# chorowski-lab/pytorch-asr

Hardware: AMD Instinct MI355X
Metric: CTC train-step frames/sec (higher is better)
Workload: dtype bf16; 1 GPU; WSJ mono-char CTC (egs/wsj/yamls/ctc.yaml shapes), DeepSpeech2 conv+4xBiLSTM-320 encoder + FSTDecoder, fwd+bwd+GradientClipping(clip 480000, skip 4.8e+06 = recipe x global_batch/16)+PolyakDecay+Adam, synthetic 40-dim x 1-channel x 1000-frame fbank; batch_per_gpu=768, global_batch=768, frames=1000, classes=49, parallelism=dp1, batch_norm=per-replica statistics, optimizer_steps=139, step_boundary=device: att_speech.fused_step (clip / skip decision + Adam, no read-back)

## Files before the change

pytorch-asr_amd/csrc/conv.hip:

```cpp
#include <type_traits>
#include "common.h"
#include "../../include/asr_amd.h"

namespace {

typedef __attribute__((ext_vector_type(8))) __bf16 bf16x8;
typedef __attribute__((ext_vector_type(16))) float f32x16;
typedef __attribute__((ext_vector_type(4))) unsigned int u32x4;
typedef __attribute__((ext_vector_type(4))) float f32x4;
typedef __attribute__((ext_vector_type(4))) __bf16 bf16x4;

constexpr int CH = 32;
constexpr int KS = 7;
constexpr int PIX = 80;
constexpr int KSTEPS = KS * KS * CH / 16;

typedef __attribute__((ext_vector_type(4))) int rsrc_words;
__device__ __forceinline__ rsrc_words conv_raw_rsrc(const void *base, unsigned bytes) {
    const unsigned long long a = (unsigned long long)base;
    rsrc_words r;
    r.x = __builtin_amdgcn_readfirstlane((int)(unsigned)a);
    r.y = __builtin_amdgcn_readfirstlane((int)((unsigned)(a >> 32) & 0xffffu));
    r.z = __builtin_amdgcn_readfirstlane((int)bytes);
    r.w = 0x00020000;
    return r;
}
__device__ __forceinline__ void conv_dma16(rsrc_words r, unsigned lds_byte, unsigned voff, unsigned soff) {
    unsigned keep;
    asm volatile("s_mov_b32 %0, m0\n\ts_mov_b32 m0, %1\n\ts_nop 0\n\t"
                 "buffer_load_dwordx4 %2, %3, %4 offen lds\n\ts_mov_b32 m0, %0"
                 : "=&s"(keep)
                 : "s"(lds_byte), "v"(voff), "s"(r), "s"(soff)
                 : "memory");
}
__device__ __forceinline__ unsigned conv_lds_addr(const void *ptr) {
    return (unsigned)(size_t)((__attribute__((address_space(3))) const void *)ptr);
}

inline int pick_row_pitch(int min_pitch, int per_row, int step, int npix, int ntiles) {
    static const int grp[2][16] = {{0, 1, 2, 3, 12, 13, 14, 15, 20, 21, 22, 23, 24, 25, 26, 27},
                                   {4, 5, 6, 7, 8, 9, 10, 11, 16, 17, 18, 19, 28, 29, 30, 31}};
    int best = min_pitch, best_cost = 1 << 30;
    for (int P = min_pitch; P <= min_pitch + 256; P += 16) {
        int cost = 0;
        for (int tile = 0; tile < ntiles; ++tile)
            for (int g = 0; g < 2; ++g) {
                int addr_of_bank[64], worst = 1, cnt[64];
                for (int b = 0; b < 64; ++b) { addr_of_bank[b] = -1; cnt[b] = 0; }
                for (int i = 0; i < 16; ++i) {
                    int m = 32 * tile + grp[g][i];
                    if (m >= npix) m = npix - 1;
                    const int r = m / per_row, w = m - r * per_row;
                    const int a = r * step * P + w * PIX;
                    for (int k = 0; k < 4; ++k) {
                        const int b = (a / 4 + k) & 63;
                        if (addr_of_bank[b] != a + 4 * k) {
                            addr_of_bank[b] = a + 4 * k;
                            if (++cnt[b] > worst) worst = cnt[b];
                        }
                    }
                }
                cost += worst;
            }
        if (cost < best_cost) { best_cost = cost; best = P; }
    }
    return best;
}

inline int conv_cu_count() {
    int dev = 0, cus = 0;
    if (hipGetDevice(&dev) != hipSuccess) return 0;
    if (hipDeviceGetAttribute(&cus, hipDeviceAttributeMultiprocessorCount, dev) != hipSuccess) return 0;
    return cus;
}

__device__ __forceinline__ void chan_partial_sums(const __bf16 *oimg, int npix, float *red, float *partial) {
    const int tid = threadIdx.x, ch = tid & 31, grp = tid >> 5;
    float s = 0.f, q = 0.f;
    int m = grp;
    for (; m + 56 < npix; m += 64) {
        float v[8];
#pragma unroll
        for (int u = 0; u < 8; ++u) v[u] = (float)oimg[(m + 8 * u) * CH + ch];
#pragma unroll
        for (int u = 0; u < 8; ++u) {
            s += v[u];
            q += v[u] * v[u];
        }
    }
    for (; m < npix; m += 8) {
        const float v = (float)oimg[m * CH + ch];
        s += v;
        q += v * v;
    }
    red[grp * 64 + ch] = s;
    red[grp * 64 + 32 + ch] = q;
    __syncthreads();
    if (tid < 64) {
        float t = 0.f;
#pragma unroll
        for (int g = 0; g < 8; ++g) t += red[g * 64 + tid];
        partial[tid] = t;
    }
}

__global__ __launch_bounds__(1024) void chan_sums_reduce_kernel(const float *partial, int nparts, double *out) {
    __shared__ double lds[1024];
    const int el = threadIdx.x & 63, way = threadIdx.x >> 6;
    double s = 0.0;
    for (int g = blockIdx.x * 16 + way; g < nparts; g += gridDim.x * 16) s += (double)partial[(size_t)g * 64 + el];
    lds[way * 64 + el] = s;
    __syncthreads();
    if (way == 0) {
        double t = 0.0;
        for (int w = 0; w < 16; ++w) t += lds[w * 64 + el];
        atomicAdd(out + el, t);
    }
}

__global__ void zero_chan_sums_kernel(double *out) { out[threadIdx.x] = 0.0; }

__global__ void conv_pack_fwd_kernel(const float *w, __bf16 *out) {
    const int i = blockIdx.x * blockDim.x + threadIdx.x;
    if (i >= KSTEPS * 64 * 8) return;
    const int j = i & 7, l = (i >> 3) & 63, s = i >> 9;
    const int k = 16 * s + 8 * (l >> 5) + j, co = l & 31;
    const int tap = k / CH, ci = k % CH, kt = tap / KS, kf = tap % KS;
    out[i] = (__bf16)w[((co * CH + ci) * KS + kt) * KS + kf];
}

#ifdef CONV_STAMPS
#define STAMP(k) do { if (p.stamps && blockIdx.x == 7 && lane == 0 && nst < 64) { p.stamps[(wave * 64 + nst) * 8 + (k)] = (long long)__builtin_amdgcn_s_memtime(); } } while (0)
#else
#define STAMP(k) do { } while (0)
#endif

struct ConvFwdParams {
    long long *stamps;
    const __bf16 *x;
    const __bf16 *wpack;
    __bf16 *y;
    float *stats;
    int B, H, W, Ho, Wo, R;
    int pitch;
};

constexpr int FWD_NT = 2, FWD_PIX = 2 * FWD_NT * 32, FWD_AD = 3;
constexpr int FWD_MAXQ = 15;

// ... 128 lines not shown
                f32x4 v = {c[4 * g], c[4 * g + 1], c[4 * g + 2], c[4 * g + 3]};
                v = KH == 0 ? v + o[g] : o[g] + v;
                bf16x4 o4 = {(__bf16)v[0], (__bf16)v[1], (__bf16)v[2], (__bf16)v[3]};
                *reinterpret_cast<bf16x4 *>(take + wr_off + (((unsigned)g ^ wr_swz) << 4)) = o4;
            }
        }
        asm volatile("" ::: "memory");
        STAMP(6);
        if (item + (int)gridDim.x < nitems) stage(item + gridDim.x, ln);
        const int rows_here = (p.Ho - ho0) < R ? (p.Ho - ho0) : R;
        const int nvalid = rows_here * Wo - 32 * tile;
        if (p.stats) {
            const unsigned ch = (unsigned)ln & 31u;
            const unsigned p0 = (unsigned)(ln >> 5) * 16u;
            float ssum = 0.f, qsum = 0.f;
#pragma unroll
            for (int k = 0; k < 16; ++k) {
                const unsigned pp = p0 + (unsigned)k;
                const unsigned short raw = *reinterpret_cast<const unsigned short *>(
                    take + pp * 64u + ((((ch >> 3) ^ (pp >> 2)) & 3u) << 4) + (ch & 7u) * 2u);
                const float v = (int)pp < nvalid ? __uint_as_float((unsigned)raw << 16) : 0.f;
                ssum += v;
                qsum += v * v;
                if ((k & 3) == 3) asm volatile("" ::: "memory");
            }
            run[ln] += ssum;
            run[64 + ln] += qsum;
        }
        asm volatile("" ::: "memory");
        STAMP(7);
        {
            const char *ybase = reinterpret_cast<const char *>(p.y) + ((size_t)b * p.Ho + ho0) * Wo * 64;
            u32x4 v[2];
#pragma unroll
            for (int it = 0; it < 2; ++it) {
                const unsigned e = (unsigned)(ln + 64 * it);
                v[it] = *reinterpret_cast<const u32x4 *>(take + ((e ^ ((e >> 4) & 3u)) << 4));
            }
#pragma unroll
            for (int it = 0; it < 2; ++it)
                conv_store16(ybase, (unsigned)(rows_here * Wo * 64), v[it], (unsigned)(2048 * tile + 16 * (ln + 64 * it)));
        }
    }
    if (p.stats) {
        const int ln = threadIdx.x & 63;
        const float a0 = run[ln & 31] + run[32 + (ln & 31)], a1 = run[64 + (ln & 31)] + run[96 + (ln & 31)];
        p.stats[((size_t)blockIdx.x * 4 + wave) * 64 + ln] = ln < 32 ? a0 : a1;
    }
}

template <int SH>
__global__ __launch_bounds__(256, 2) void conv7x7c32_fwd_kernel(ConvFwdParams p) {
    extern __shared__ char smem[];
    const int lane = threadIdx.x & 63;
    const int wave = __builtin_amdgcn_readfirstlane(threadIdx.x >> 6);
    if ((wave & 1) == 0) conv_fwd_wave<SH, 0>(p, smem, lane, wave);
    else conv_fwd_wave<SH, 1>(p, smem, lane, wave);
}


__global__ void conv_pack_dgrad_kernel(const float *w, __bf16 *out) {
    const int i = blockIdx.x * blockDim.x + threadIdx.x;
    if (i >= KSTEPS * 64 * 8) return;
    const int jj = i & 7, l = (i >> 3) & 63, s = i >> 9;
    const int r = s < 42 ? 0 : (s < 70 ? 1 : 2);
    const int sl = s - (r == 0 ? 0 : (r == 1 ? 42 : 70));
    const int j = sl / 14, rem = sl % 14, kf = rem >> 1, cp = rem & 1;
    const int co = cp * 16 + 8 * (l >> 5) + jj, ci = l & 31, kt = r + 3 * j;
    out[i] = (__bf16)w[((co * CH + ci) * KS + kt) * KS + kf];
}

struct ConvDgradParams {
    long long *stamps;
    const __bf16 *dy;
    const __bf16 *wpack;
    __bf16 *dx;
    int B, H, W, Ho, Wo, Rq;
    int pitch;
    int flip;
};

constexpr int DG_NT = 6, DG_PIX = DG_NT * 32, DG_AD = 2;

template <int NS, int S0>
__device__ __forceinline__ void conv_dgrad_part(const char *img, const unsigned (&pixbase)[DG_NT], int pitch,
                                                const bf16x8 (&bf)[28], f32x16 (&acc)[DG_NT]) {
    constexpr int N = NS * DG_NT;
    auto frag = [&](int idx) {
        const int s = idx / DG_NT, i = idx % DG_NT;
        const int sl = S0 + s;
        const int j = sl / 14, rem = sl % 14, kf = rem >> 1, cp = rem & 1;
        const unsigned off = (unsigned)((2 - j) * pitch + (6 - kf) * PIX + cp * 32);
        return *reinterpret_cast<const bf16x8 *>(img + pixbase[i] + off);
    };
    bf16x8 a[DG_AD];
#pragma unroll
    for (int d = 0; d < DG_AD; ++d) a[d] = frag(d);
#pragma unroll
    for (int idx = 0; idx < N; ++idx) {
        acc[idx % DG_NT] = __builtin_amdgcn_mfma_f32_32x32x16_bf16(bf[idx / DG_NT], a[idx % DG_AD],
                                                                   idx < DG_NT ? f32x16{} : acc[idx % DG_NT], 0, 0, 0);
        if (idx + DG_AD < N) a[idx % DG_AD] = frag(idx + DG_AD);
    }
#pragma unroll
    for (int d = 0; d < DG_AD; ++d) __builtin_amdgcn_sched_group_barrier(0x100, 1, 0);
#pragma unroll
    for (int idx = 0; idx < N; ++idx) {
        __builtin_amdgcn_sched_group_barrier(0x008, 1, 0);
        if (idx + DG_AD < N) __builtin_amdgcn_sched_group_barrier(0x100, 1, 0);
    }
}

template <int ROLE>
__device__ __forceinline__ void conv_dgrad_wave(const ConvDgradParams &p, char *smem, int lane, int wave) {
    constexpr int NS = ROLE < 2 ? 21 : 28;
    constexpr int FIRST = ROLE == 0 ? 0 : (ROLE == 1 ? 21 : (ROLE == 2 ? 42 : 70));
    constexpr int R = ROLE < 2 ? 0 : ROLE - 1;
    constexpr int HT = DG_NT / 2;
    constexpr int NT = ROLE < 2 ? HT : DG_NT, T0 = ROLE == 1 ? HT : 0;
    constexpr int GIVE0 = ROLE == 0 ? HT : 0;
    constexpr int SLOTS = 14;
    const int W = p.W, Wo = p.Wo, Rq = p.Rq;
    const unsigned img_bytes = (unsigned)(Rq + 2) * (unsigned)p.pitch;
    bf16x8 bf[28];
    {
        const bf16x8 *src = reinterpret_cast<const bf16x8 *>(p.wpack) + (size_t)FIRST * 64 + lane;
#pragma unroll
        for (int s = 0; s < NS; ++s) bf[s] = src[(size_t)s * 64];
    }
    unsigned tab[SLOTS];
    if (ROLE < 2) {
#pragma unroll
        for (int kk = 0; kk < SLOTS; ++kk) {
            const unsigned beta = (unsigned)(SLOTS * ROLE + kk) * 1024u + (unsigned)lane * 16u;
            const unsigned row = beta / (unsigned)p.pitch, rem = beta - row * (unsigned)p.pitch;
            const unsigned col = (rem * 52429u) >> 22, within = rem - col * 80u;
            const int wo = (int)col - 6;
            const bool ok = beta < img_bytes && within < 64u && wo >= 0 && wo < Wo;
            tab[kk] = ok ? (row * (unsigned)Wo + (unsigned)wo) * 64u + within : 0xC0000000u;
        }
    }
    unsigned pixbase[DG_NT];
    const int npix = Rq * W;
#pragma unroll
    for (int i = 0; i < DG_NT; ++i) {
        int m = 32 * i + (lane & 31);
        if (m >= npix) m = npix - 1;
        const int q = m / W, w = m - q * W;
        pixbase[i] = (unsigned)(q * p.pitch + w * PIX + (lane >> 5) * 16);
    }
    const int nq = (p.H + 2) / 3;
    const int tiles = (nq + Rq - 1) / Rq, nitems = tiles * p.B;
    const int nslots = (int)((img_bytes + 1023u) / 1024u);
    constexpr int HALF = HT * 4 * 64 * 16;
    char *epi = smem + nslots * 1024;
    char *part_out = epi + (ROLE == 0 ? 0 : HALF);
    char *part_in = epi + (ROLE == 0 ? HALF : 0);
    char *ocls = ROLE == 0 ? epi + HALF : ROLE == 1 ? epi - T0 * 2048 : epi + 2 * HALF + (R - 1) * DG_PIX * 64;
    const unsigned img_lds = conv_lds_addr(smem);
    const unsigned item_bytes = (unsigned)(p.Ho * Wo * 64);
    auto stage = [&](int it) {
        const int b = it / tiles, q0 = (it - b * tiles) * Rq;
        const rsrc_words yR = conv_raw_rsrc(reinterpret_cast<const char *>(p.dy) + (size_t)b * item_bytes, item_bytes);
        const unsigned base = (unsigned)((q0 - 2) * Wo * 64);
#pragma unroll
        for (int kk = 0; kk < SLOTS; ++kk)
            if (SLOTS * ROLE + kk < nslots)
                conv_dma16(yR, (unsigned)__builtin_amdgcn_readfirstlane((int)(img_lds + (SLOTS * ROLE + kk) * 1024u)),
                           tab[kk] + base, 0u);
    };
    if (ROLE < 2 && (int)blockIdx.x < nitems) stage(blockIdx.x);
    const unsigned wr_base = (unsigned)((lane & 31) * 64 + ((lane >> 5) << 3));
    const unsigned wr_swz = (unsigned)((lane >> 2) & 3);
    const unsigned qmagic = 65536u / (unsigned)W + 1u;
    const int cls_chunks = Rq * W * 4;
    int nst = 0;
    for (int item = blockIdx.x; item < nitems; item += gridDim.x, ++nst) {
        const int b = item / tiles, q0 = (item - b * tiles) * Rq;
        STAMP(0);
        if (ROLE < 2) asm volatile("s_waitcnt vmcnt(0)" ::: "memory");
        __syncthreads();
        f32x16 acc[DG_NT];
        STAMP(1);
        conv_dgrad_part<NS, ROLE == 1 ? 21 : 0>(smem, pixbase, p.pitch, bf, acc);
        STAMP(2);
        if (ROLE < 2) {
#pragma unroll
            for (int i = 0; i < HT; ++i)
#pragma unroll
                for (int g = 0; g < 4; ++g) {
                    const f32x16 &c = acc[GIVE0 + i];
                    *reinterpret_cast<f32x4 *>(part_out + ((i * 4 + g) * 64 + lane) * 16) =
                        f32x4{c[4 * g], c[4 * g + 1], c[4 * g + 2], c[4 * g + 3]};
                }
        }
        STAMP(3);
        __syncthreads();
        STAMP(4);
        if (ROLE < 2 && item + (int)gridDim.x < nitems) stage(item + gridDim.x);
        {
            constexpr int E = NT * 4, RD = ROLE < 2 ? E / 2 : E;
#pragma unroll
            for (int e0 = 0; e0 < E; e0 += RD) {
                f32x4 o[ROLE < 2 ? RD : 1];
                if (ROLE < 2) {
#pragma unroll
                    for (int k = 0; k < RD; ++k)
                        o[k] = *reinterpret_cast<const f32x4 *>(part_in + ((e0 + k) * 64 + lane) * 16);
                    asm volatile("s_waitcnt lgkmcnt(0)" ::: "memory");
                }
#pragma unroll
                for (int k = 0; k < RD; ++k) {
                    const int i = (e0 + k) / 4, g = (e0 + k) % 4;
                    const f32x16 &c = acc[T0 + i];
                    f32x4 v = {c[4 * g], c[4 * g + 1], c[4 * g + 2], c[4 * g + 3]};
                    if (ROLE < 2) v += o[k];
                    bf16x4 o4 = {(__bf16)v[0], (__bf16)v[1], (__bf16)v[2], (__bf16)v[3]};
                    *reinterpret_cast<bf16x4 *>(ocls + (T0 + i) * 2048 + wr_base + (((unsigned)g ^ wr_swz) << 4)) = o4;
                }
            }
        }
        STAMP(5);
        {
            char *xb = reinterpret_cast<char *>(p.dx) + ((size_t)b * p.H + 3 * q0 + R) * W * 64;
            const int qlim = (p.H - R + 2) / 3 - q0;
            int e0 = T0 * 128 + lane;
            asm volatile("" : "+v"(e0));
#pragma unroll
            for (int rd = 0; rd < NT * 2; rd += 6) {
                u32x4 v[6];
#pragma unroll
                for (int it = 0; it < 6; ++it) {
                    const unsigned e = (unsigned)(e0 + 64 * (rd + it)), m = e >> 2;
                    v[it] = *reinterpret_cast<const u32x4 *>(ocls + ((e ^ ((m >> 2) & 3u)) << 4));
                }
#pragma unroll
                for (int it = 0; it < 6; ++it) {
                    const unsigned e = (unsigned)(e0 + 64 * (rd + it)), m = e >> 2, q = (m * qmagic) >> 16;
                    if ((int)e < cls_chunks && (int)q < qlim)
                        *reinterpret_cast<u32x4 *>(xb + (size_t)(e * 16u + q * (unsigned)(2 * W * 64))) = v[it];
                }
            }
        }
        STAMP(6); STAMP(7);
    }
}

__global__ __launch_bounds__(256, 2) void conv7x7c32_dgrad_s3_kernel(ConvDgradParams p) {
    extern __shared__ char smem[];
    const int lane = threadIdx.x & 63;
    const int wave = __builtin_amdgcn_readfirstlane(threadIdx.x >> 6);
    const int role = __builtin_amdgcn_readfirstlane(p.flip && blockIdx.x >= (gridDim.x >> 1) ? 3 - wave : wave);
    if (role == 0) conv_dgrad_wave<0>(p, smem, lane, wave);
    else if (role == 1) conv_dgrad_wave<1>(p, smem, lane, wave);
    else if (role == 2) conv_dgrad_wave<2>(p, smem, lane, wave);
    else conv_dgrad_wave<3>(p, smem, lane, wave);
}


typedef __attribute__((ext_vector_type(4))) short s16x4;
typedef __attribute__((ext_vector_type(8))) short s16x8;
typedef __attribute__((address_space(3))) s16x4 lds_s16x4;

__device__ __forceinline__ bf16x8 tr_frag(const char *addr) {
    const s16x4 lo = __builtin_amdgcn_ds_read_tr16_b64_v4i16((lds_s16x4 *)(addr));
    const s16x4 hi = __builtin_amdgcn_ds_read_tr16_b64_v4i16((lds_s16x4 *)(addr + 4 * PIX));
    s16x8 v;
    v.s0 = lo.x; v.s1 = lo.y; v.s2 = lo.z; v.s3 = lo.w;
    v.s4 = hi.x; v.s5 = hi.y; v.s6 = hi.z; v.s7 = hi.w;
    return __builtin_bit_cast(bf16x8, v);
}

constexpr int WGRAD_WGS = 256;
constexpr int WGRAD_NT = 448;
constexpr int NX_MAX = 8, ND_MAX = 3;

struct ConvWgradParams {
    const __bf16 *x, *dy;
    float *partial;
    int B, H, W, Ho, Wo, KW;
    int rows;
};

__global__ __launch_bounds__(WGRAD_NT) void conv7x7c32_wgrad_s3_kernel(ConvWgradParams p) {
    extern __shared__ char smem[];
    const int tid = threadIdx.x, lane = tid & 63;
    const int wave = __builtin_amdgcn_readfirstlane(tid >> 6);
    const int W = p.W, Wo = p.Wo, KW = p.KW, Wd = 16 * KW, rows = p.rows;
    const int xrows = 3 * (rows - 1) + KS;
    char *ximg = smem;
    char *dimg = smem + (size_t)(xrows * W + 24) * PIX;
    const int kt = wave;
    f32x16 acc[KS];
#pragma unroll
    for (int f = 0; f < KS; ++f)
#pragma unroll
        for (int j = 0; j < 16; ++j) acc[f][j] = 0.f;
    const unsigned lane_off = (unsigned)((8 * (lane >> 5) + ((lane & 15) >> 2)) * PIX +
                                         (16 * ((lane >> 4) & 1) + 4 * (lane & 3)) * 2);
    for (int i = tid; i < 24 * PIX / 4; i += WGRAD_NT)
        reinterpret_cast<unsigned *>(ximg + (size_t)xrows * W * PIX)[i] = 0u;
    const int chunks_per_utt = (p.Ho + rows - 1) / rows;
    const int nchunks = p.B * chunks_per_utt;
    const int nx = xrows * W * 4, nd = rows * Wd * 4;
    u32x4 sx[NX_MAX], sd[ND_MAX];
    const unsigned wmagic = (1u << 20) / (unsigned)W + 1u, dmagic = (1u << 20) / (unsigned)Wd + 1u;
    auto fetch = [&](int c) {
        const int b = c / chunks_per_utt, ho0 = (c - b * chunks_per_utt) * rows;
        const char *xb = reinterpret_cast<const char *>(p.x) + (size_t)b * p.H * W * 64;
        const char *yb = reinterpret_cast<const char *>(p.dy) + (size_t)b * p.Ho * Wo * 64;
#pragma unroll
        for (int k = 0; k < NX_MAX; ++k) {
            const int i = tid + k * WGRAD_NT;
            const int pix = i >> 2, part = i & 3, row = (int)(((unsigned)pix * wmagic) >> 20);
            u32x4 v = {0u, 0u, 0u, 0u};
            if (i < nx && 3 * ho0 + row < p.H)
                v = *reinterpret_cast<const u32x4 *>(xb + ((size_t)(3 * ho0) * W + pix) * 64 + part * 16);
            sx[k] = v;
        }
#pragma unroll
        for (int k = 0; k < ND_MAX; ++k) {
            const int i = tid + k * WGRAD_NT;
            const int pix = i >> 2, part = i & 3, row = (int)(((unsigned)pix * dmagic) >> 20), wo = pix - row * Wd;
            u32x4 v = {0u, 0u, 0u, 0u};
            if (i < nd && ho0 + row < p.Ho && wo < Wo)
                v = *reinterpret_cast<const u32x4 *>(yb + ((size_t)(ho0 + row) * Wo + wo) * 64 + part * 16);
            sd[k] = v;
        }
    };
    auto stage = [&]() {
#pragma unroll
        for (int k = 0; k < NX_MAX; ++k) {
            const int i = tid + k * WGRAD_NT;
            if (i < nx) *reinterpret_cast<u32x4 *>(ximg + (i >> 2) * PIX + (i & 3) * 16) = sx[k];
        }
#pragma unroll
        for (int k = 0; k < ND_MAX; ++k) {
            const int i = tid + k * WGRAD_NT;
            if (i < nd) *reinterpret_cast<u32x4 *>(dimg + (i >> 2) * PIX + (i & 3) * 16) = sd[k];
        }
    };
    int c = blockIdx.x;
    if (c < nchunks) fetch(c);
    __syncthreads();
    if (c < nchunks) stage();
    __syncthreads();
    for (; c < nchunks; c += gridDim.x) {
        const int next = c + gridDim.x;
        if (next < nchunks) fetch(next);
        for (int r = 0; r < rows; ++r) {
            for (int ks = 0; ks < KW; ++ks) {
                const bf16x8 a = tr_frag(dimg + (size_t)(r * Wd + 16 * ks) * PIX + lane_off);
                const char *xr = ximg + (size_t)((3 * r + kt) * W + 16 * ks) * PIX + lane_off;
#pragma unroll
                for (int f = 0; f < KS; ++f) {
                    const bf16x8 bb = tr_frag(xr + f * PIX);
                    acc[f] = __builtin_amdgcn_mfma_f32_32x32x16_bf16(a, bb, acc[f], 0, 0, 0);
                }
            }
        }
        __syncthreads();
        if (next < nchunks) stage();
        __syncthreads();
    }
    float *out = p.partial + (size_t)blockIdx.x * 49 * 1024;
#pragma unroll
    for (int f = 0; f < KS; ++f)
#pragma unroll
        for (int j = 0; j < 16; ++j) out[((kt * KS + f) * 16 + j) * 64 + lane] = acc[f][j];
}

__device__ __forceinline__ float partial_sum(const float *partial, int nparts, int n, float *lds) {
    const int el = threadIdx.x & 63, part = threadIdx.x >> 6, ways = blockDim.x >> 6;
    const int e = blockIdx.x * 64 + el;
    float s = 0.f;
    if (e < n)
        for (int g = part; g < nparts; g += ways) s += partial[(size_t)g * n + e];
    lds[part * 64 + el] = s;
    __syncthreads();
    float t = 0.f;
    for (int w = 0; w < ways; ++w) t += lds[w * 64 + el];
    return t;
}

__global__ __launch_bounds__(1024) void conv_wgrad_reduce_kernel(const float *partial, int nwg, float *dw) {
    __shared__ float lds4[1024];
    const float s = partial_sum(partial, nwg, 49 * 1024, lds4);
    const int e = blockIdx.x * 64 + (threadIdx.x & 63);
    if (threadIdx.x >= 64 || e >= 49 * 1024) return;
    const int tap = e >> 10, j = (e >> 6) & 15, l = e & 63;
    const int co = (j & 3) + 8 * (j >> 2) + 4 * (l >> 5), ci = l & 31;
    dw[(co * CH + ci) * 49 + tap] = s;
}


constexpr int C1_ROWS = 16;

__global__ void conv1_pack_kernel(const float *w, __bf16 *out) {
    const int i = blockIdx.x * blockDim.x + threadIdx.x;
    if (i >= 4 * 64 * 8) return;
    const int j = i & 7, l = (i >> 3) & 63, s = i >> 9;
    const int kt = 2 * s + (l >> 5), kf = j, co = l & 31;
    out[i] = (kt < KS && kf < KS) ? (__bf16)w[(co * KS + kt) * KS + kf] : (__bf16)0.f;
}

struct Conv1Params {
    const float *x;
    const __bf16 *wpack;
    __bf16 *y;
    float *partial;
    int B, T, F, To, Fo;
};

__device__ __forceinline__ void conv1_stage_windows(const Conv1Params &p, int b, int t0, int nrows,
                                                    char *wimg, int tid, int nt) {
    const float *xb = p.x + (size_t)b * p.T * p.F;
    const unsigned fmagic = (1u << 20) / (unsigned)p.Fo + 1u;
    for (int i = tid; i < nrows * p.Fo; i += nt) {
        const unsigned row = ((unsigned)i * fmagic) >> 20, fo = (unsigned)i - row * (unsigned)p.Fo;
        const int t = t0 - 6 + (int)row;
        bf16x8 v = {};
        if (t >= 0 && t < p.T) {
            const float2 *src = reinterpret_cast<const float2 *>(xb + (size_t)t * p.F + 2 * fo);
            const bool whole = 2 * (int)fo + 7 < p.F;
#pragma unroll
            for (int j = 0; j < 4; ++j) {
                float2 f2;
                if (j < 3 || whole) f2 = src[j];
                else f2 = float2{reinterpret_cast<const float *>(src)[6], 0.f};
                v[2 * j] = (__bf16)f2.x;
                v[2 * j + 1] = (__bf16)f2.y;
            }
        }
        *reinterpret_cast<bf16x8 *>(wimg + (size_t)i * 16) = v;
    }
}

__global__ __launch_bounds__(256) void conv1_fwd_kernel(Conv1Params p) {
    extern __shared__ char smem[];
    const int tid = threadIdx.x, lane = tid & 63;
    const int wave = __builtin_amdgcn_readfirstlane(tid >> 6);
// ... 450 lines not shown
    hipEventRecord(stamp_ev[0], s);
}
static void stamp_dump(const char *name, long long *d, hipStream_t s) {
    if (!d) return;
    hipEventRecord(stamp_ev[1], s);
    hipDeviceSynchronize();
    float ms = 0;
    hipEventElapsedTime(&ms, stamp_ev[0], stamp_ev[1]);
    static long long h[4 * 64 * 8];
    hipMemcpy(h, d, sizeof(h), hipMemcpyDeviceToHost);
    for (int w = 0; w < 4; ++w)
        for (int lo = 2; lo < 30; lo += 14) {
            double avg[9] = {0};
            for (int it = lo; it < lo + 12; ++it) {
                for (int k = 1; k < 8; ++k) avg[k] += (double)(h[(w * 64 + it) * 8 + k] - h[(w * 64 + it) * 8 + k - 1]) / 12;
                avg[8] += (double)(h[(w * 64 + it + 1) * 8] - h[(w * 64 + it) * 8]) / 12;
            }
            fprintf(stderr, "%s wave %d items %d..%d avg:", name, w, lo, lo + 11);
            for (int k = 1; k < 8; ++k) fprintf(stderr, " %6.0f", avg[k]);
            fprintf(stderr, "  | total %.0f\n", avg[8]);
        }
    fprintf(stderr, "%s kernel %.1f us; items 0..30 of block 7 took %lld ticks\n", name, ms * 1e3, h[30 * 8] - h[0]);
}
#endif

extern "C" int64_t asr_conv7x7c32_workspace_bytes(void) {
    return (int64_t)KSTEPS * 64 * 8 * 2 * 2 + (int64_t)WGRAD_WGS * 49 * 1024 * 4 + 256;
}

struct ConvFwdPlan { int Ho, Wo, R, pitch; size_t lds; };
static int conv_fwd_plan(int B, int H, int W, int stride_h, ConvFwdPlan *pl) {
    if (B <= 0 || H < KS || W < KS) return ASR_EINVAL;
    if (stride_h != 1 && stride_h != 3) return ASR_EUNSUPPORTED;
    const int Ho = (H - KS) / stride_h + 1, Wo = W - KS + 1;
    if (Wo > 48) return ASR_EUNSUPPORTED;
    int R = FWD_PIX / Wo;
    if (R > 16) R = 16;
    const int pitch = pick_row_pitch(W * PIX, Wo, stride_h, R * Wo, 2 * FWD_NT);
    const size_t img = ((size_t)(stride_h * (R - 1) + KS) * pitch + 1023) / 1024 * 1024;
    if ((int64_t)H * W * 64 >= (1ll << 31)) return ASR_EUNSUPPORTED;
    if (img > (size_t)4 * FWD_MAXQ * 1024) return ASR_EUNSUPPORTED;
    const size_t lds = img + img / 8 + 4 * 4096 + 2048;
    if (lds > 80 * 1024) return ASR_EUNSUPPORTED;
    pl->Ho = Ho; pl->Wo = Wo; pl->R = R; pl->pitch = pitch; pl->lds = lds;
    return ASR_OK;
}

struct ConvDgradPlan { int Ho, Wo, Rq, pitch; size_t lds; };
static int conv_dgrad_plan(int B, int H, int W, int stride_h, ConvDgradPlan *pl) {
    if (B <= 0 || H < KS || W < KS) return ASR_EINVAL;
    if (stride_h != 3) return ASR_EUNSUPPORTED;
    const int Ho = (H - KS) / stride_h + 1, Wo = W - KS + 1;
    if (W > 48) return ASR_EUNSUPPORTED;
    int Rq = DG_PIX / W;
    if (Rq > 16) Rq = 16;
    const int pitch = pick_row_pitch((Wo + 12) * PIX, W, 1, Rq * W, DG_NT);
    const size_t img = ((size_t)(Rq + 2) * pitch + 1023) / 1024 * 1024;
    if ((int64_t)B * Ho * Wo * 64 >= (1ll << 31)) return ASR_EUNSUPPORTED;
    const size_t epi = (size_t)DG_NT * 4 * 64 * 16 + (size_t)2 * DG_PIX * CH * 2;
    const size_t lds = img + epi;
    if (lds > 80 * 1024 || img > 28 * 1024) return ASR_EUNSUPPORTED;
    pl->Ho = Ho; pl->Wo = Wo; pl->Rq = Rq; pl->pitch = pitch; pl->lds = lds;
    return ASR_OK;
}

struct ConvWgradPlan { int Ho, Wo, KW, rows; size_t lds; };
static int conv_wgrad_plan(int B, int H, int W, int stride_h, ConvWgradPlan *pl) {
    if (B <= 0 || H < KS || W < KS) return ASR_EINVAL;
    if (stride_h != 3) return ASR_EUNSUPPORTED;
    const int Ho = (H - KS) / stride_h + 1, Wo = W - KS + 1;
    if (Wo > 48) return ASR_EUNSUPPORTED;
    const int KW = (Wo + 15) / 16;
    int rows = 8;
    size_t lds = 0;
    for (; rows >= 1; rows >>= 1) {
        const int xrows = 3 * (rows - 1) + KS;
        lds = (size_t)(xrows * W + 24) * PIX + (size_t)rows * 16 * KW * PIX;
        if (lds <= 72 * 1024 && xrows * W * 4 <= NX_MAX * WGRAD_NT && rows * 16 * KW * 4 <= ND_MAX * WGRAD_NT)
            break;
    }
    if (rows < 1) return ASR_EUNSUPPORTED;
    pl->Ho = Ho; pl->Wo = Wo; pl->KW = KW; pl->rows = rows; pl->lds = lds;
    return ASR_OK;
}

extern "C" int asr_conv7x7c32_supported(int B, int H, int W, int stride_h) {
    ConvFwdPlan f;
    ConvDgradPlan d;
    ConvWgradPlan g;
    return conv_fwd_plan(B, H, W, stride_h, &f) == ASR_OK && conv_dgrad_plan(B, H, W, stride_h, &d) == ASR_OK &&
           conv_wgrad_plan(B, H, W, stride_h, &g) == ASR_OK;
}

extern "C" int asr_conv7x7c32_fwd_bf16(const void *x, const float *w, int B, int H, int W,
                                       int stride_h, void *y, double *chan_sums, void *workspace,
                                       int64_t workspace_bytes, void *stream) {
    if (B <= 0 || H < KS || W < KS) return ASR_EINVAL;
    if (!x || !w || !y || !workspace || workspace_bytes < asr_conv7x7c32_workspace_bytes())
        return ASR_EINVAL;
    ConvFwdPlan pl;
    const int rc = conv_fwd_plan(B, H, W, stride_h, &pl);
    if (rc != ASR_OK) return rc;
    const int Ho = pl.Ho, Wo = pl.Wo, R = pl.R, pitch = pl.pitch;
    const size_t lds = pl.lds;
    hipStream_t s = (hipStream_t)stream;
    __bf16 *wpack = (__bf16 *)workspace;
    hipLaunchKernelGGL(conv_pack_fwd_kernel, dim3((KSTEPS * 64 * 8 + 255) / 256), dim3(256), 0, s, w, wpack);
    ConvFwdParams p;
    p.x = (const __bf16 *)x; p.wpack = wpack; p.y = (__bf16 *)y;
    p.B = B; p.H = H; p.W = W; p.Ho = Ho; p.Wo = Wo; p.R = R; p.pitch = pitch;
    const int nitems = ((Ho + R - 1) / R) * B;
    int wgs = 2 * conv_cu_count();
    if (wgs <= 0) wgs = 512;
    if (wgs > nitems) wgs = nitems;
    const dim3 grid(wgs);
    p.stats = chan_sums ? (float *)((char *)workspace + (size_t)KSTEPS * 64 * 8 * 2 * 2) : nullptr;
    if (chan_sums && (int64_t)wgs * 4 * 64 * 4 > (int64_t)WGRAD_WGS * 49 * 1024 * 4) return ASR_EUNSUPPORTED;
    void (*kern)(ConvFwdParams) = stride_h == 3 ? conv7x7c32_fwd_kernel<3> : conv7x7c32_fwd_kernel<1>;
    if (lds > 64 * 1024 &&
        hipFuncSetAttribute((const void *)kern, hipFuncAttributeMaxDynamicSharedMemorySize, (int)lds) != hipSuccess)
        return ASR_EUNSUPPORTED;
#ifdef CONV_STAMPS
    p.stamps = stamp_buf();
    stamp_begin(s);
#else
    p.stamps = nullptr;
#endif
    hipLaunchKernelGGL(kern, grid, dim3(256), lds, s, p);
#ifdef CONV_STAMPS
    stamp_dump("fwd", p.stamps, s);
#endif
    if (chan_sums) {
        hipLaunchKernelGGL(zero_chan_sums_kernel, dim3(1), dim3(64), 0, s, chan_sums);
        hipLaunchKernelGGL(chan_sums_reduce_kernel, dim3(64), dim3(1024), 0, s, p.stats, wgs * 4, chan_sums);
    }
    return hipGetLastError() == hipSuccess ? ASR_OK : ASR_ELAUNCH;
}

extern "C" int asr_conv7x7c32_bwd_data_bf16(const void *dy, const float *w, int B, int H, int W,
                                            int stride_h, void *dx, void *workspace,
                                            int64_t workspace_bytes, void *stream) {
    if (B <= 0 || H < KS || W < KS) return ASR_EINVAL;
    if (!dy || !w || !dx || !workspace || workspace_bytes < asr_conv7x7c32_workspace_bytes())
        return ASR_EINVAL;
    ConvDgradPlan pl;
    const int rc = conv_dgrad_plan(B, H, W, stride_h, &pl);
    if (rc != ASR_OK) return rc;
    const int Ho = pl.Ho, Wo = pl.Wo, Rq = pl.Rq, pitch = pl.pitch;
    const size_t lds = pl.lds;
    hipStream_t s = (hipStream_t)stream;
    __bf16 *wpack = (__bf16 *)workspace + (size_t)KSTEPS * 64 * 8;
    hipLaunchKernelGGL(conv_pack_dgrad_kernel, dim3((KSTEPS * 64 * 8 + 255) / 256), dim3(256), 0, s, w, wpack);
    ConvDgradParams p;
    p.dy = (const __bf16 *)dy; p.wpack = wpack; p.dx = (__bf16 *)dx;
    p.B = B; p.H = H; p.W = W; p.Ho = Ho; p.Wo = Wo; p.Rq = Rq; p.pitch = pitch;
    const int nq = (H + 2) / 3;
    const int nitems = ((nq + Rq - 1) / Rq) * B;
    int wgs = 2 * conv_cu_count();
    if (wgs <= 0) wgs = 512;
    p.flip = wgs <= nitems;
    if (wgs > nitems) wgs = nitems;
    const dim3 grid(wgs);
    if (lds > 64 * 1024 &&
        hipFuncSetAttribute((const void *)conv7x7c32_dgrad_s3_kernel,
                            hipFuncAttributeMaxDynamicSharedMemorySize, (int)lds) != hipSuccess)
        return ASR_EUNSUPPORTED;
#ifdef CONV_STAMPS
    p.stamps = stamp_buf();
    stamp_begin(s);
#else
    p.stamps = nullptr;
#endif
    hipLaunchKernelGGL(conv7x7c32_dgrad_s3_kernel, grid, dim3(256), lds, s, p);
#ifdef CONV_STAMPS
    stamp_dump("dgrad", p.stamps, s);
#endif
    return hipGetLastError() == hipSuccess ? ASR_OK : ASR_ELAUNCH;
}

extern "C" int asr_conv7x7c32_wgrad_bf16(const void *x, const void *dy, int B, int H, int W,
                                         int stride_h, float *dw, void *workspace,
                                         int64_t workspace_bytes, void *stream) {
    if (B <= 0 || H < KS || W < KS) return ASR_EINVAL;
    if (!x || !dy || !dw || !workspace || workspace_bytes < asr_conv7x7c32_workspace_bytes())
        return ASR_EINVAL;
    ConvWgradPlan pl;
    const int rc = conv_wgrad_plan(B, H, W, stride_h, &pl);
    if (rc != ASR_OK) return rc;
    const int Ho = pl.Ho, Wo = pl.Wo, KW = pl.KW, rows = pl.rows;
    const size_t lds = pl.lds;
    hipStream_t s = (hipStream_t)stream;
    ConvWgradParams p;
    p.x = (const __bf16 *)x; p.dy = (const __bf16 *)dy;
    p.partial = (float *)((char *)workspace + (size_t)KSTEPS * 64 * 8 * 2 * 2);
    p.B = B; p.H = H; p.W = W; p.Ho = Ho; p.Wo = Wo; p.KW = KW; p.rows = rows;
    const int chunks = B * ((Ho + rows - 1) / rows);
    const int nwg = chunks < WGRAD_WGS ? chunks : WGRAD_WGS;
    if (lds > 64 * 1024 &&
        hipFuncSetAttribute((const void *)conv7x7c32_wgrad_s3_kernel,
                            hipFuncAttributeMaxDynamicSharedMemorySize, (int)lds) != hipSuccess)
        return ASR_EUNSUPPORTED;
    hipLaunchKernelGGL(conv7x7c32_wgrad_s3_kernel, dim3(nwg), dim3(WGRAD_NT), lds, s, p);
    hipLaunchKernelGGL(conv_wgrad_reduce_kernel, dim3(49 * 1024 / 64), dim3(256), 0, s,
                       p.partial, nwg, dw);
    return hipGetLastError() == hipSuccess ? ASR_OK : ASR_ELAUNCH;
}

extern "C" int64_t asr_conv1_7x7s2_workspace_bytes(void) {
    return 4 * 64 * 8 * 2 + (int64_t)(1 << 17) * 64 * 4 + 256;
}

static int conv1_shapes(int B, int T, int F, int *To, int *Fo) {
    if (B <= 0 || T <= 0 || F < KS) return ASR_EINVAL;
    *To = T + 2 * 6 - KS + 1;
    *Fo = (F - KS) / 2 + 1;
    if (*Fo > 64) return ASR_EUNSUPPORTED;
    return ASR_OK;
}

static int conv1_fwd_check(int B, int T, int F, int want_sums, int *To, int *Fo, size_t *lds) {
    const int rc = conv1_shapes(B, T, F, To, Fo);
    if (rc != ASR_OK) return rc;
    const int64_t wgs = (int64_t)((*To + C1_ROWS - 1) / C1_ROWS) * B;
    if (want_sums && wgs * 64 * 4 > asr_conv1_7x7s2_workspace_bytes() - 4 * 64 * 8 * 2 - 256)
        return ASR_EUNSUPPORTED;
    const int ntiles = (C1_ROWS * *Fo + 31) / 32;
    *lds = (size_t)(C1_ROWS + 8) * *Fo * 16 + (size_t)ntiles * 32 * CH * 2 + 512 * 4;
    if (*lds > 64 * 1024) return ASR_EUNSUPPORTED;
    return ASR_OK;
}

static int conv1_wgrad_check(int B, int T, int F, int bn, int *To, int *Fo, size_t *lds) {
    const int rc = conv1_shapes(B, T, F, To, Fo);
    if (rc != ASR_OK) return rc;
    *lds = (size_t)(C1_ROWS + 8) * *Fo * 16 + (size_t)C1_ROWS * *Fo * PIX + (bn ? CH * 8 * 4 : 0);
    if (*lds < 4 * 2 * 1024 * 4) *lds = 4 * 2 * 1024 * 4;
    if (*lds > 64 * 1024) return ASR_EUNSUPPORTED;
    if (bn && !asr_conv1_7x7s2_wgrad_bn_supported(F)) return ASR_EUNSUPPORTED;
    return ASR_OK;
}

extern "C" int asr_conv1_7x7s2_fwd(const float *x, const float *w, int B, int T, int F, void *y,
                                   double *chan_sums, void *workspace, int64_t workspace_bytes,
                                   void *stream) {
    int To, Fo;
    size_t lds;
    int rc = conv1_shapes(B, T, F, &To, &Fo);
    if (rc != ASR_OK) return rc;
    if (!x || !w || !y || !workspace || workspace_bytes < asr_conv1_7x7s2_workspace_bytes())
        return ASR_EINVAL;
    rc = conv1_fwd_check(B, T, F, chan_sums != nullptr, &To, &Fo, &lds);
    if (rc != ASR_OK) return rc;
    hipStream_t s = (hipStream_t)stream;
    __bf16 *wpack = (__bf16 *)workspace;
    hipLaunchKernelGGL(conv1_pack_kernel, dim3(8), dim3(256), 0, s, w, wpack);
    Conv1Params p;
    p.x = x; p.wpack = wpack; p.y = (__bf16 *)y;
    p.B = B; p.T = T; p.F = F; p.To = To; p.Fo = Fo;
    const dim3 grid((To + C1_ROWS - 1) / C1_ROWS, B);
    p.partial = chan_sums ? (float *)((char *)workspace + 4 * 64 * 8 * 2) : nullptr;
    hipLaunchKernelGGL(conv1_fwd_kernel, grid, dim3(256), lds, s, p);
    if (chan_sums) {
        hipLaunchKernelGGL(zero_chan_sums_kernel, dim3(1), dim3(64), 0, s, chan_sums);
        hipLaunchKernelGGL(chan_sums_reduce_kernel, dim3(64), dim3(1024), 0, s, p.partial, (int)(grid.x * grid.y), chan_sums);
    }
    return hipGetLastError() == hipSuccess ? ASR_OK : ASR_ELAUNCH;
}

static void conv1_wgrad_sizes(int Fo, int *di, int *wpt) {
    *di = (C1_ROWS * Fo * 4 + 255) / 256;
    *wpt = ((C1_ROWS + 8) * Fo + 255) / 256;
}

static int conv1_wgrad_launch(const float *x, const void *dy, int B, int T, int F, float *dw,
                              void *workspace, int64_t workspace_bytes, const Conv1BnParams *bn,
                              void *stream) {
    int To, Fo;
    size_t lds;
    int rc = conv1_shapes(B, T, F, &To, &Fo);
    if (rc != ASR_OK) return rc;
    if (!x || !dy || !dw || !workspace || workspace_bytes < asr_conv1_7x7s2_workspace_bytes())
        return ASR_EINVAL;
    rc = conv1_wgrad_check(B, T, F, bn != nullptr, &To, &Fo, &lds);
    if (rc != ASR_OK) return rc;
    hipStream_t s = (hipStream_t)stream;
// ... 160 lines not shown
```

Measured before the change: 37.15 million frames/s.

## Add W=17 dgrad specialization skipping zero taps and dense wgrad kernel

Adds a specialized dgrad kernel for the 17-wide conv2 shape. It uses a w-major pixel layout, picks its pitch with a bank-conflict model, and drops MFMA steps whose filter taps fall entirely outside the valid output columns, with the kept steps chosen at compile time. It also adds a dense wgrad kernel that stages contiguous rows and reads them with transposing LDS loads. That kernel uses a different row-chunking plan, which aims to cut padding waste in both backward convolutions. Both paths are on by default, can be turned off with environment switches, and add code size and shape-specific complexity.

```diff
diff --git a/pytorch-asr_amd/csrc/conv.hip b/pytorch-asr_amd/csrc/conv.hip
--- a/pytorch-asr_amd/csrc/conv.hip
+++ b/pytorch-asr_amd/csrc/conv.hip
@@ -37,7 +37,8 @@
     return (unsigned)(size_t)((__attribute__((address_space(3))) const void *)ptr);
 }
 
-inline int pick_row_pitch(int min_pitch, int per_row, int step, int npix, int ntiles) {
+template <class Addr>
+inline int pick_pitch(int min_pitch, int npix, int ntiles, Addr addr) {
     static const int grp[2][16] = {{0, 1, 2, 3, 12, 13, 14, 15, 20, 21, 22, 23, 24, 25, 26, 27},
                                    {4, 5, 6, 7, 8, 9, 10, 11, 16, 17, 18, 19, 28, 29, 30, 31}};
     int best = min_pitch, best_cost = 1 << 30;
@@ -50,8 +51,7 @@
                 for (int i = 0; i < 16; ++i) {
                     int m = 32 * tile + grp[g][i];
                     if (m >= npix) m = npix - 1;
-                    const int r = m / per_row, w = m - r * per_row;
-                    const int a = r * step * P + w * PIX;
+                    const int a = addr(m, P);
                     for (int k = 0; k < 4; ++k) {
                         const int b = (a / 4 + k) & 63;
                         if (addr_of_bank[b] != a + 4 * k) {
@@ -65,6 +65,15 @@
         if (cost < best_cost) { best_cost = cost; best = P; }
     }
     return best;
+}
+inline int pick_row_pitch(int min_pitch, int per_row, int step, int npix, int ntiles) {
+    return pick_pitch(min_pitch, npix, ntiles, [=](int m, int P) {
+        const int r = m / per_row, w = m - r * per_row;
+        return r * step * P + w * PIX;
+    });
+}
+inline int pick_row_pitch_wmajor(int min_pitch, int rows, int npix, int ntiles) {
+    return pick_pitch(min_pitch, npix, ntiles, [=](int m, int P) { return (m % rows) * P + (m / rows) * PIX; });
 }
 
 inline int conv_cu_count() {
@@ -359,6 +368,57 @@
 
 constexpr int DG_NT = 6, DG_PIX = DG_NT * 32, DG_AD = 2;
 
+constexpr int DG17_W = 17, DG17_WO = 11, DG17_RQ = 11, DG17_NPIX = DG17_RQ * DG17_W;
+constexpr bool dg17_keep(int i, int kf) {
+    const int last = 32 * i + 31 < DG17_NPIX ? 32 * i + 31 : DG17_NPIX - 1;
+    const int wlo = 32 * i / DG17_RQ, whi = last / DG17_RQ;
+    return kf <= whi && kf >= wlo - (DG17_WO - 1);
+}
+template <int N> struct DgSeq { int n; int s[N], i[N]; bool first[N]; };
+template <int NS, int S0>
+constexpr DgSeq<NS * DG_NT> dg17_seq() {
+    DgSeq<NS * DG_NT> q{};
+    bool seen[DG_NT] = {};
+    for (int s = 0; s < NS; ++s)
+        for (int i = 0; i < DG_NT; ++i) {
+            const int kf = ((S0 + s) % 14) >> 1;
+            if (!dg17_keep(i, kf)) continue;
+            q.s[q.n] = s; q.i[q.n] = i; q.first[q.n] = !seen[i];
+            seen[i] = true;
+            ++q.n;
+        }
+    return q;
+}
+
+template <int NS, int S0>
+__device__ __forceinline__ void conv_dgrad17_part(const char *img, const unsigned (&pixbase)[DG_NT], int pitch,
+                                                  const bf16x8 (&bf)[28], f32x16 (&acc)[DG_NT]) {
+    constexpr DgSeq<NS * DG_NT> Q = dg17_seq<NS, S0>();
+    constexpr int N = Q.n;
+    auto frag = [&](int idx) {
+        const int sl = S0 + Q.s[idx], i = Q.i[idx];
+        const int j = sl / 14, rem = sl % 14, kf = rem >> 1, cp = rem & 1;
+        const unsigned off = (unsigned)((2 - j) * pitch + (6 - kf) * PIX + cp * 32);
+        return *reinterpret_cast<const bf16x8 *>(img + pixbase[i] + off);
+    };
+    bf16x8 a[DG_AD];
+#pragma unroll
+    for (int d = 0; d < DG_AD; ++d) a[d] = frag(d);
+#pragma unroll
+    for (int idx = 0; idx < N; ++idx) {
+        acc[Q.i[idx]] = __builtin_amdgcn_mfma_f32_32x32x16_bf16(bf[Q.s[idx]], a[idx % DG_AD],
+                                                                Q.first[idx] ? f32x16{} : acc[Q.i[idx]], 0, 0, 0);
+        if (idx + DG_AD < N) a[idx % DG_AD] = frag(idx + DG_AD);
+    }
+#pragma unroll
+    for (int d = 0; d < DG_AD; ++d) __builtin_amdgcn_sched_group_barrier(0x100, 1, 0);
+#pragma unroll
+    for (int idx = 0; idx < N; ++idx) {
+        __builtin_amdgcn_sched_group_barrier(0x008, 1, 0);
+        if (idx + DG_AD < N) __builtin_amdgcn_sched_group_barrier(0x100, 1, 0);
+    }
+}
+
 template <int NS, int S0>
 __device__ __forceinline__ void conv_dgrad_part(const char *img, const unsigned (&pixbase)[DG_NT], int pitch,
                                                 const bf16x8 (&bf)[28], f32x16 (&acc)[DG_NT]) {
@@ -388,7 +448,7 @@
     }
 }
 
-template <int ROLE>
+template <int ROLE, bool W17 = false>
 __device__ __forceinline__ void conv_dgrad_wave(const ConvDgradParams &p, char *smem, int lane, int wave) {
     constexpr int NS = ROLE < 2 ? 21 : 28;
     constexpr int FIRST = ROLE == 0 ? 0 : (ROLE == 1 ? 21 : (ROLE == 2 ? 42 : 70));
@@ -423,7 +483,7 @@
     for (int i = 0; i < DG_NT; ++i) {
         int m = 32 * i + (lane & 31);
         if (m >= npix) m = npix - 1;
-        const int q = m / W, w = m - q * W;
+        const int q = W17 ? m % DG17_RQ : m / W, w = W17 ? m / DG17_RQ : m - q * W;
         pixbase[i] = (unsigned)(q * p.pitch + w * PIX + (lane >> 5) * 16);
     }
     const int nq = (p.H + 2) / 3;
@@ -459,7 +519,8 @@
         __syncthreads();
         f32x16 acc[DG_NT];
         STAMP(1);
-        conv_dgrad_part<NS, ROLE == 1 ? 21 : 0>(smem, pixbase, p.pitch, bf, acc);
+        if constexpr (W17) conv_dgrad17_part<NS, ROLE == 1 ? 21 : 0>(smem, pixbase, p.pitch, bf, acc);
+        else conv_dgrad_part<NS, ROLE == 1 ? 21 : 0>(smem, pixbase, p.pitch, bf, acc);
         STAMP(2);
         if (ROLE < 2) {
 #pragma unroll
@@ -513,9 +574,16 @@
                 }
 #pragma unroll
                 for (int it = 0; it < 6; ++it) {
-                    const unsigned e = (unsigned)(e0 + 64 * (rd + it)), m = e >> 2, q = (m * qmagic) >> 16;
-                    if ((int)e < cls_chunks && (int)q < qlim)
-                        *reinterpret_cast<u32x4 *>(xb + (size_t)(e * 16u + q * (unsigned)(2 * W * 64))) = v[it];
+                    const unsigned e = (unsigned)(e0 + 64 * (rd + it)), m = e >> 2;
+                    if constexpr (W17) {
+                        const unsigned w = (m * (65536u / DG17_RQ + 1u)) >> 16, q = m - w * DG17_RQ;
+                        if ((int)e < cls_chunks && (int)q < qlim)
+                            *reinterpret_cast<u32x4 *>(xb + (size_t)((((3u * q) * DG17_W + w) * 4u + (e & 3u)) * 16u)) = v[it];
+                    } else {
+                        const unsigned q = (m * qmagic) >> 16;
+                        if ((int)e < cls_chunks && (int)q < qlim)
+                            *reinterpret_cast<u32x4 *>(xb + (size_t)(e * 16u + q * (unsigned)(2 * W * 64))) = v[it];
+                    }
                 }
             }
         }
@@ -532,6 +600,17 @@
     else if (role == 1) conv_dgrad_wave<1>(p, smem, lane, wave);
     else if (role == 2) conv_dgrad_wave<2>(p, smem, lane, wave);
     else conv_dgrad_wave<3>(p, smem, lane, wave);
+}
+
+__global__ __launch_bounds__(256, 2) void conv7x7c32_dgrad_s3_w17_kernel(ConvDgradParams p) {
+    extern __shared__ char smem[];
+    const int lane = threadIdx.x & 63;
+    const int wave = __builtin_amdgcn_readfirstlane(threadIdx.x >> 6);
+    const int role = __builtin_amdgcn_readfirstlane(p.flip && blockIdx.x >= (gridDim.x >> 1) ? 3 - wave : wave);
+    if (role == 0) conv_dgrad_wave<0, true>(p, smem, lane, wave);
+    else if (role == 1) conv_dgrad_wave<1, true>(p, smem, lane, wave);
+    else if (role == 2) conv_dgrad_wave<2, true>(p, smem, lane, wave);
+    else conv_dgrad_wave<3, true>(p, smem, lane, wave);
 }
 
 
@@ -634,6 +713,126 @@
                     const bf16x8 bb = tr_frag(xr + f * PIX);
                     acc[f] = __builtin_amdgcn_mfma_f32_32x32x16_bf16(a, bb, acc[f], 0, 0, 0);
                 }
+            }
+        }
+        __syncthreads();
+        if (next < nchunks) stage();
+        __syncthreads();
+    }
+    float *out = p.partial + (size_t)blockIdx.x * 49 * 1024;
+#pragma unroll
+    for (int f = 0; f < KS; ++f)
+#pragma unroll
+        for (int j = 0; j < 16; ++j) out[((kt * KS + f) * 16 + j) * 64 + lane] = acc[f][j];
+}
+
+__device__ __forceinline__ bf16x8 tr_frag2(const char *lo_addr, const char *hi_addr) {
+    const s16x4 lo = __builtin_amdgcn_ds_read_tr16_b64_v4i16((lds_s16x4 *)(lo_addr));
+    const s16x4 hi = __builtin_amdgcn_ds_read_tr16_b64_v4i16((lds_s16x4 *)(hi_addr));
+    s16x8 v;
+    v.s0 = lo.x; v.s1 = lo.y; v.s2 = lo.z; v.s3 = lo.w;
+    v.s4 = hi.x; v.s5 = hi.y; v.s6 = hi.z; v.s7 = hi.w;
+    return __builtin_bit_cast(bf16x8, v);
+}
+
+__global__ __launch_bounds__(WGRAD_NT) void conv7x7c32_wgrad_dense_s3_kernel(ConvWgradParams p) {
+    extern __shared__ char smem[];
+    const int tid = threadIdx.x, lane = tid & 63;
+    const int wave = __builtin_amdgcn_readfirstlane(tid >> 6);
+    const int W = p.W, Wo = p.Wo, rows = p.rows;
+    const int xrows = 3 * (rows - 1) + KS;
+    const int npix = rows * Wo, npd = (npix + 15) & ~15;
+    char *ximg = smem;
+    char *dimg = smem + (size_t)xrows * W * PIX;
+    const int kt = wave;
+    f32x16 acc[KS];
+#pragma unroll
+    for (int f = 0; f < KS; ++f)
+#pragma unroll
+        for (int j = 0; j < 16; ++j) acc[f][j] = 0.f;
+    const int kpix = 8 * (lane >> 5) + ((lane & 15) >> 2);
+    const unsigned choff = (unsigned)((16 * ((lane >> 4) & 1) + 4 * (lane & 3)) * 2);
+    const int chunks_per_utt = (p.Ho + rows - 1) / rows;
+    const int nchunks = p.B * chunks_per_utt;
+    const int nx = xrows * W * 4, nd = npd * 4;
+    u32x4 sx[NX_MAX], sd[ND_MAX];
+    const unsigned wmagic = (1u << 20) / (unsigned)W + 1u, omagic = (1u << 20) / (unsigned)Wo + 1u;
+    const unsigned rowskip = (unsigned)(3 * W - Wo);
+    auto fetch = [&](int c) {
+        const int b = c / chunks_per_utt, ho0 = (c - b * chunks_per_utt) * rows;
+        const char *xb = reinterpret_cast<const char *>(p.x) + (size_t)b * p.H * W * 64;
+        const char *yb = reinterpret_cast<const char *>(p.dy) + ((size_t)b * p.Ho + ho0) * Wo * 64;
+        const int left = (p.Ho - ho0) * Wo;
+#pragma unroll
+        for (int k = 0; k < NX_MAX; ++k) {
+            const int i = tid + k * WGRAD_NT;
+            const int pix = i >> 2, part = i & 3, row = (int)(((unsigned)pix * wmagic) >> 20);
+            u32x4 v = {0u, 0u, 0u, 0u};
+            if (i < nx && 3 * ho0 + row < p.H)
+                v = *reinterpret_cast<const u32x4 *>(xb + ((size_t)(3 * ho0) * W + pix) * 64 + part * 16);
+            sx[k] = v;
+        }
+#pragma unroll
+        for (int k = 0; k < ND_MAX; ++k) {
+            const int i = tid + k * WGRAD_NT;
+            const int pix = i >> 2;
+            u32x4 v = {0u, 0u, 0u, 0u};
+            if (i < nd && pix < npix && pix < left)
+                v = *reinterpret_cast<const u32x4 *>(yb + (size_t)i * 16);
+            sd[k] = v;
+        }
+    };
+    auto stage = [&]() {
+#pragma unroll
+        for (int k = 0; k < NX_MAX; ++k) {
+            const int i = tid + k * WGRAD_NT;
+            if (i < nx) *reinterpret_cast<u32x4 *>(ximg + (i >> 2) * PIX + (i & 3) * 16) = sx[k];
+        }
+#pragma unroll
+        for (int k = 0; k < ND_MAX; ++k) {
+            const int i = tid + k * WGRAD_NT;
+            if (i < nd) *reinterpret_cast<u32x4 *>(dimg + (i >> 2) * PIX + (i & 3) * 16) = sd[k];
+        }
+    };
+    const char *xtap = ximg + (size_t)kt * W * PIX + choff;
+    const char *dtap = dimg + kpix * PIX + choff;
+    auto read_a = [&](int ks) { return tr_frag2(dtap + 16 * ks * PIX, dtap + (16 * ks + 4) * PIX); };
+    auto window = [&](int pix) {
+        const unsigned q = (unsigned)(pix < npix ? pix : npix - 1);
+        return xtap + (q + ((q * omagic) >> 20) * rowskip) * PIX;
+    };
+    int c = blockIdx.x;
+    if (c < nchunks) fetch(c);
+    __syncthreads();
+    if (c < nchunks) stage();
+    __syncthreads();
+    for (; c < nchunks; c += gridDim.x) {
+        const int next = c + gridDim.x;
+        if (next < nchunks) fetch(next);
+        const int ho0 = (c % chunks_per_utt) * rows;
+        const int rows_here = p.Ho - ho0 < rows ? p.Ho - ho0 : rows;
+        const int nks = (rows_here * Wo + 15) >> 4;
+        bf16x8 a = read_a(0), b[KS];
+        {
+            const char *x0 = window(kpix), *x1 = window(kpix + 4);
+#pragma unroll
+            for (int f = 0; f < KS; ++f) b[f] = tr_frag2(x0 + f * PIX, x1 + f * PIX);
+        }
+        for (int ks = 0; ks < nks; ++ks) {
+            const int kn = ks + 1 < nks ? ks + 1 : ks;
+            const bf16x8 an = read_a(kn);
+            const char *x0 = window(16 * kn + kpix), *x1 = window(16 * kn + kpix + 4);
+#pragma unroll
+            for (int f = 0; f < KS; ++f) {
+                acc[f] = __builtin_amdgcn_mfma_f32_32x32x16_bf16(a, b[f], acc[f], 0, 0, 0);
+                b[f] = tr_frag2(x0 + f * PIX, x1 + f * PIX);
+            }
+            a = an;
+            __builtin_amdgcn_sched_group_barrier(0x100, 2, 0);
+#pragma unroll
+            for (int f = 0; f < KS; ++f) {
+                __builtin_amdgcn_sched_group_barrier(0x008, 1, 0);
+                __builtin_amdgcn_sched_group_barrier(0x100, 2, 0);
             }
         }
         __syncthreads();
@@ -1250,6 +1449,33 @@
     if (rows < 1) return ASR_EUNSUPPORTED;
     pl->Ho = Ho; pl->Wo = Wo; pl->KW = KW; pl->rows = rows; pl->lds = lds;
     return ASR_OK;
+}
+
+struct ConvWgradDensePlan { int rows; size_t lds; };
+static bool conv_wgrad_dense_plan(int W, int Wo, ConvWgradDensePlan *pl) {
+    for (int rows = 16; rows >= 1; rows >>= 1) {
+        const int xrows = 3 * (rows - 1) + KS, npd = (rows * Wo + 15) & ~15;
+        const size_t lds = (size_t)(xrows * W + npd) * PIX;
+        if (lds <= 128 * 1024 && xrows * W * 4 <= NX_MAX * WGRAD_NT && npd * 4 <= ND_MAX * WGRAD_NT) {
+            pl->rows = rows; pl->lds = lds;
+            return true;
+        }
+    }
+    return false;
+}
+
+static bool conv_dgrad17_plan(int W, const ConvDgradPlan &g, ConvDgradPlan *pl) {
+    if (W != DG17_W || g.Wo != DG17_WO || g.Rq != DG17_RQ) return false;
+    *pl = g;
+    pl->pitch = pick_row_pitch_wmajor((g.Wo + 12) * PIX, g.Rq, g.Rq * W, DG_NT);
+    const size_t img = ((size_t)(g.Rq + 2) * pl->pitch + 1023) / 1024 * 1024;
+    pl->lds = img + (size_t)DG_NT * 4 * 64 * 16 + (size_t)2 * DG_PIX * CH * 2;
+    return pl->lds <= 80 * 1024 && img <= 28 * 1024;
+}
+
+static bool conv_switch_off(const char *name) {
+    const char *v = getenv(name);
+    return v && v[0] == '0' && v[1] == 0;
 }
 
 extern "C" int asr_conv7x7c32_supported(int B, int H, int W, int stride_h) {
@@ -1314,6 +1540,12 @@
     ConvDgradPlan pl;
     const int rc = conv_dgrad_plan(B, H, W, stride_h, &pl);
     if (rc != ASR_OK) return rc;
+    void (*kern)(ConvDgradParams) = conv7x7c32_dgrad_s3_kernel;
+    ConvDgradPlan pl17;
+    if (!conv_switch_off("ASR_CONV_DGRAD_SKIP") && conv_dgrad17_plan(W, pl, &pl17)) {
+        kern = conv7x7c32_dgrad_s3_w17_kernel;
+        pl = pl17;
+    }
     const int Ho = pl.Ho, Wo = pl.Wo, Rq = pl.Rq, pitch = pl.pitch;
     const size_t lds = pl.lds;
     hipStream_t s = (hipStream_t)stream;
@@ -1330,8 +1562,7 @@
     if (wgs > nitems) wgs = nitems;
     const dim3 grid(wgs);
     if (lds > 64 * 1024 &&
-        hipFuncSetAttribute((const void *)conv7x7c32_dgrad_s3_kernel,
-                            hipFuncAttributeMaxDynamicSharedMemorySize, (int)lds) != hipSuccess)
+        hipFuncSetAttribute((const void *)kern, hipFuncAttributeMaxDynamicSharedMemorySize, (int)lds) != hipSuccess)
         return ASR_EUNSUPPORTED;
 #ifdef CONV_STAMPS
     p.stamps = stamp_buf();
@@ -1339,7 +1570,7 @@
 #else
     p.stamps = nullptr;
 #endif
-    hipLaunchKernelGGL(conv7x7c32_dgrad_s3_kernel, grid, dim3(256), lds, s, p);
+    hipLaunchKernelGGL(kern, grid, dim3(256), lds, s, p);
 #ifdef CONV_STAMPS
     stamp_dump("dgrad", p.stamps, s);
 #endif
@@ -1362,13 +1593,26 @@
     p.x = (const __bf16 *)x; p.dy = (const __bf16 *)dy;
     p.partial = (float *)((char *)workspace + (size_t)KSTEPS * 64 * 8 * 2 * 2);
     p.B = B; p.H = H; p.W = W; p.Ho = Ho; p.Wo = Wo; p.KW = KW; p.rows = rows;
-    const int chunks = B * ((Ho + rows - 1) / rows);
+    void (*kern)(ConvWgradParams) = conv7x7c32_wgrad_s3_kernel;
+    size_t kern_lds = lds;
+    ConvWgradDensePlan dp;
+    if (!conv_switch_off("ASR_CONV_WGRAD_DENSE") && conv_wgrad_dense_plan(W, Wo, &dp)) {
+        void (*dense)(ConvWgradParams) = conv7x7c32_wgrad_dense_s3_kernel;
+        if (dp.lds <= 64 * 1024 ||
+            hipFuncSetAttribute((const void *)dense, hipFuncAttributeMaxDynamicSharedMemorySize, (int)dp.lds) == hipSuccess) {
+            kern = dense;
+            kern_lds = dp.lds;
+            p.rows = dp.rows;
+        } else {
+            (void)hipGetLastError();
+        }
+    }
+    const int chunks = B * ((Ho + p.rows - 1) / p.rows);
     const int nwg = chunks < WGRAD_WGS ? chunks : WGRAD_WGS;
-    if (lds > 64 * 1024 &&
-        hipFuncSetAttribute((const void *)conv7x7c32_wgrad_s3_kernel,
-                            hipFuncAttributeMaxDynamicSharedMemorySize, (int)lds) != hipSuccess)
+    if (kern_lds > 64 * 1024 &&
+        hipFuncSetAttribute((const void *)kern, hipFuncAttributeMaxDynamicSharedMemorySize, (int)kern_lds) != hipSuccess)
         return ASR_EUNSUPPORTED;
-    hipLaunchKernelGGL(conv7x7c32_wgrad_s3_kernel, dim3(nwg), dim3(WGRAD_NT), lds, s, p);
+    hipLaunchKernelGGL(kern, dim3(nwg), dim3(WGRAD_NT), kern_lds, s, p);
     hipLaunchKernelGGL(conv_wgrad_reduce_kernel, dim3(49 * 1024 / 64), dim3(256), 0, s,
                        p.partial, nwg, dw);
     return hipGetLastError() == hipSuccess ? ASR_OK : ASR_ELAUNCH;
```

Measured after the change: 37.34 million frames/s, median of 5. About the same (+0.5%).
